# adobe-research/DiffusionHandles

Hardware: AMD Instinct MI355X
Metric: guided-denoise steps/sec at 512x512 (SD2-depth) (higher is better)
Workload: dtype f16; 1 GPU; single 512x512 edit per GPU, SD2-depth (865.9M params, seeded random weights), guided phase: 3 x (fwd + energy + bwd-to-latent) + CFG fwd (B=2) + DDIM step; resolution=512, edits_per_gpu=1, correspondences=24906, parallelism=independent edits, one process per GPU, no collectives

## Files before the change

diffusionhandles_amd/_lib.py:

```python
import ctypes
import os

import torch

_HERE = os.path.dirname(os.path.abspath(__file__))
LIB_PATH = os.environ.get("DIFFHANDLES_LIB") or os.path.join(_HERE, "libdiffhandles_hip.so")
_LIB = None

c_p = ctypes.c_void_p
c_i = ctypes.c_int
c_f = ctypes.c_float
c_d = ctypes.c_double
c_sz = ctypes.c_size_t


class UNetConfig(ctypes.Structure):
    _fields_ = [("in_channels", c_i), ("out_channels", c_i), ("n_levels", c_i),
                ("block_out_channels", c_i * 4), ("layers_per_block", c_i), ("heads", c_i * 4),
                ("cross_attention_dim", c_i), ("norm_groups", c_i), ("sample_size", c_i),
                ("text_len", c_i), ("max_batch", c_i), ("dtype", c_i), ("max_diff_batch", c_i)]


class VAEConfig(ctypes.Structure):
    _fields_ = [("latent_channels", c_i), ("out_channels", c_i), ("block_out_channels", c_i * 4),
# ... 97 lines not shown
    "dh_adam_step_scaled_batch": (c_i, [c_p, c_p, c_p, c_p, c_p, c_p, c_f, c_f, c_f, c_f, c_i, c_i, c_i, c_p]),
    "dh_latent_update_guarded": (c_i, [c_p, c_p, c_p, c_i, c_i, c_f, c_i, c_i, c_p, c_i, c_i, c_p, c_p, c_i, c_i, c_p]),
    "dh_ddim_cfg_step_flagged": (c_i, [c_p, c_p, c_p, c_p, c_f, c_f, c_f, c_i, c_i, c_p, c_i, c_i, c_p]),
}

c_l = ctypes.c_long
DEBUG_SIGNATURES = {
    "dh_dbg_gemm": (c_i, [c_i, c_p, c_l, c_p, c_i, c_i, c_i, c_i, c_i, c_i, c_i, c_i, c_i, c_i, c_i, c_p, c_p, c_i, c_i,
                          c_p, c_l, c_p, c_l, c_i, c_p, c_sz, c_p]),
    "dh_dbg_gemm_groupnorm": (c_i, [c_i, c_p, c_l, c_p, c_i, c_i, c_i, c_i, c_i, c_i, c_i, c_p, c_p, c_p, c_sz, c_i, c_i, c_p, c_p, c_f, c_i,
                                    c_p, c_p, c_p, ctypes.POINTER(c_i), c_p]),
    "dh_dbg_gemm_groupnorm_bwd": (c_i, [c_i, c_p, c_l, c_p, c_i, c_i, c_i, c_i, c_i, c_i, c_i, c_p, c_p, c_sz, c_i, c_i, c_p, c_p, c_p, c_p, c_i,
                                        c_p, c_p, ctypes.POINTER(c_i), c_p]),
    "dh_dbg_gemm_groupnorm_res": (c_i, [c_i, c_p, c_l, c_p, c_i, c_i, c_i, c_i, c_i, c_i, c_i, c_p, c_p, c_l, c_p, c_p, c_sz, c_i, c_i, c_p, c_p,
                                    c_f, c_i, c_p, c_p, c_p, ctypes.POINTER(c_i), c_p]),
    "dh_dbg_gemm_groupnorm_bwd_res": (c_i, [c_i, c_p, c_l, c_p, c_i, c_i, c_i, c_i, c_i, c_i, c_i, c_p, c_l, c_p, c_p, c_sz, c_i, c_i, c_p, c_p, c_p,
                                        c_p, c_i, c_p, c_p, ctypes.POINTER(c_i), c_p]),
    "dh_dbg_concat_groupnorm": (c_i, [c_i, c_p, c_i, c_p, c_i, c_p, c_i, c_i, c_i, c_p, c_p, c_f, c_i, c_p, c_p, c_p, c_p]),
    "dh_dbg_gemm_last_tile": (c_i, [ctypes.POINTER(c_i)]),
    "dh_dbg_unet_concat_ops": (c_i, [ctypes.POINTER(UNetConfig), ctypes.POINTER(c_i), c_i, ctypes.POINTER(c_i)]),
    "dh_dbg_gemm_lnfold": (c_i, [c_i, c_p, c_l, c_p, c_i, c_i, c_i, c_p, c_p, c_p, c_f, c_p, c_l, c_p]),
    "dh_dbg_gemm_glu": (c_i, [c_i, c_i, c_p, c_l, c_p, c_i, c_i, c_i, c_p, c_p, c_p, c_p, c_p, c_p]),
    "dh_dbg_gemm_glub_split": (c_i, [c_i, c_p, c_l, c_p, c_i, c_i, c_i, c_i, c_p, c_l, c_i, c_p, c_p, ctypes.POINTER(c_i), c_p]),
    "dh_dbg_unet_ff_fold": (c_i, [c_p, c_i, ctypes.POINTER(c_i), ctypes.POINTER(c_i), c_p, c_p, c_p]),
    "dh_dbg_gemm_family": (c_i, [c_i]),
    "dh_dbg_gemm_stage": (c_i, [c_i]),
    "dh_dbg_gemm_xattn": (c_i, [c_i, c_p, c_l, c_p, c_i, c_i, c_i, c_p, c_p, c_p, c_p, c_f, c_p, c_p, c_p, c_l, c_p, c_p, c_i, c_i, c_i,
                                ctypes.POINTER(c_i), c_p]),
    "dh_dbg_gemm_xattn_dq": (c_i, [c_i, c_p, c_l, c_p, c_i, c_i, c_i, c_p, c_p, c_p, c_p, c_l, c_p, c_p, c_p, c_i, c_i, ctypes.POINTER(c_i), c_p]),
    "dh_dbg_gemm_xattn_carried": (c_i, [ctypes.POINTER(c_i), ctypes.POINTER(ctypes.c_longlong)]),
    "dh_dbg_gemm_pp_variant": (c_i, [c_i, c_p]),
    "dh_dbg_gemm_pp_ablate": (c_i, [c_i]),
    "dh_dbg_gemm_pp_persist": (c_i, [c_i]),
    "dh_dbg_gemm_pp_glu": (c_i, [c_i]),
    "dh_dbg_gemm_pp_plan": (c_i, [c_i, c_i, c_i, c_i, c_i, c_i, c_sz, ctypes.POINTER(c_i), ctypes.POINTER(c_i), ctypes.POINTER(c_i)]),
    "dh_dbg_touch_tiled": (c_i, [c_sz, c_p]),
    "dh_dbg_groupnorm": (c_i, [c_i, c_p, c_p, c_p, c_p, c_p, c_p, c_p, c_p, c_i, c_i, c_i, c_i, c_f, c_i, c_i, c_p]),
    "dh_dbg_layernorm": (c_i, [c_i, c_p, c_p, c_p, c_p, c_p, c_p, c_p, c_p, c_i, c_i, c_f, c_p]),
    "dh_dbg_geglu": (c_i, [c_i, c_p, c_p, c_p, c_p, c_i, c_i, c_p]),
    "dh_dbg_attention": (c_i, [c_i, c_p, c_l, c_p, c_p, c_l, c_p, c_l, c_p, c_p, c_p, c_p, c_p, c_p, c_i, c_i, c_i, c_i, c_p]),
    "dh_dbg_attention_bwd_pair": (c_i, [c_i, c_p, c_l, c_p, c_p, c_l, c_p, c_l, c_p, c_p, c_p, c_p, c_p, c_p, c_i, c_i, c_i, c_i, c_p, c_p]),
    "dh_dbg_pool2x2": (c_i, [c_i, c_p, c_p, c_i, c_i, c_i, c_i, c_i, c_p]),
    "dh_dbg_ellipse_offsets": (c_i, [c_i, ctypes.POINTER(ctypes.c_int32), c_i, ctypes.POINTER(c_i)]),
    "dh_dbg_lane_ops": (c_i, [c_p, c_p, c_p, c_p]),
    "dh_dbg_cg_limits": (c_i, [ctypes.POINTER(c_i)]),
    "dh_dbg_cg_max_iter": (c_i, [c_i]),
}


def lib():
    global _LIB
    if _LIB is None:
        if not os.path.exists(LIB_PATH):
            raise RuntimeError(
                f"native HIP library not found at {LIB_PATH}; build it with "
                "`python -c 'import __graft_entry__ as g; g.build()'` (there is no CPU fallback)")
        handle = ctypes.CDLL(LIB_PATH)
        missing = []
        for name, (res, args) in list(SIGNATURES.items()) + list(DEBUG_SIGNATURES.items()):
            try:
# ... 38 lines not shown
```

diffusionhandles_amd/csrc/debug_api.cpp:

```cpp
#include <stdlib.h>

#include "unet_kernels.h"
using namespace dh;

static void* g_dbg_tiled = nullptr;

__global__ void k_dbg_touch(const uint4* p, size_t n16, unsigned* sink) {
  unsigned acc = 0;
  for (size_t i = (size_t)blockIdx.x * blockDim.x + threadIdx.x; i < n16; i += (size_t)gridDim.x * blockDim.x) { const uint4 v = p[i]; acc ^= v.x ^ v.y ^ v.z ^ v.w; }
  if (acc == 0x9e3779b9u && sink) sink[0] = acc;
}
extern "C" int dh_dbg_touch_tiled(size_t bytes, void* stream) {
  DH_REQUIRE(g_dbg_tiled != nullptr, "no tiled weights yet (call dh_dbg_gemm first)");
  hipLaunchKernelGGL(k_dbg_touch, dim3(512), dim3(256), 0, (hipStream_t)stream, (const uint4*)g_dbg_tiled, bytes / 16, (unsigned*)nullptr);
  DH_LAUNCH_CHECK();
  return DH_OK;
}

extern "C" int dh_dbg_gemm(int dtype, const void* A, long lda, const void* W, int M, int N, int K, int mode, int Hin,
                           int Win, int Cin, int Hout, int Wout, int stride, int up, const float* bias,
                           const float* rowvec, int rowvec_ld, int rows_per_batch, const void* R, long ldr, void* C,
                           long ldc, int act_silu, float* partial, size_t partial_elems, void* stream) {
  DH_REQUIRE(A && W && C && K % 64 == 0 && N % 64 == 0, "bad arguments (N, K must be multiples of 64)");
  void*& tiled = g_dbg_tiled;
// ... 197 lines not shown
  if (need > tiled_cap) {
    if (tiled) (void)hipFree(tiled);
    DH_CHECK_HIP(hipMalloc(&tiled, need));
    tiled_cap = need;
  }
  DH_CHECK_HIP(hipMemsetAsync(tiled, 0, need, (hipStream_t)stream));
  launch_tile_weights(dtype, W, tiled, N, K, (hipStream_t)stream);
  GemmArgs g;
  g.A = A; g.lda = lda; g.W = tiled; g.M = M; g.N = N; g.K = K; g.mode = A_DENSE;
  g.glub_x = x; g.glub_dx = dx; g.glub_f = F;
  g.C = C; g.ldc = ldc;
  if (accumulate) { g.R = C; g.ldr = ldc; }
  launch_gemm(dtype, g, (hipStream_t)stream);
  if (tile) dh_dbg_gemm_last_tile(tile);
  DH_LAUNCH_CHECK();
  return DH_OK;
}
extern "C" int dh_dbg_groupnorm(int dtype, const void* x, const float* gamma, const float* beta, void* y, float* stats,
                                const void* dy, void* dx, float* scratch, int B, int HW, int C, int G, float eps,
                                int silu, int accumulate, void* stream) {
  launch_groupnorm_fwd(dtype, x, gamma, beta, y, stats, scratch, B, HW, C, G, eps, silu, (hipStream_t)stream);
  if (dy && dx)
    launch_groupnorm_bwd(dtype, x, dy, gamma, beta, stats, dx, scratch, B, HW, C, G, silu, accumulate, (hipStream_t)stream);
  DH_LAUNCH_CHECK();
  return DH_OK;
}
extern "C" int dh_dbg_layernorm(int dtype, const void* x, const float* gamma, const float* beta, void* y, float* stats,
                                const void* dy, const void* add, void* dx, int rows, int C, float eps, void* stream) {
  launch_layernorm_fwd(dtype, x, gamma, beta, y, stats, rows, C, eps, (hipStream_t)stream);
  if (dy && dx) launch_layernorm_bwd(dtype, x, dy, gamma, stats, add, dx, rows, C, (hipStream_t)stream);
  DH_LAUNCH_CHECK();
  return DH_OK;
}
extern "C" int dh_dbg_geglu(int dtype, const void* x, void* y, const void* dy, void* dx, int rows, int F, void* stream) {
  launch_geglu_fwd(dtype, x, y, rows, F, (hipStream_t)stream);
  if (dy && dx) launch_geglu_bwd(dtype, x, dy, dx, rows, F, (hipStream_t)stream);
  DH_LAUNCH_CHECK();
  return DH_OK;
}
extern "C" int dh_dbg_attention(int dtype, const void* q, long ldq, const void* k, const void* v, long ldk, void* o,
                                long ldo, float* lse, const void* d_o, float* delta, void* dq, void* dk, void* dv,
                                int B, int H, int Nq, int Nk, void* stream) {
  hipStream_t st = (hipStream_t)stream;
  launch_attention_fwd(dtype, q, ldq, k, v, ldk, o, ldo, lse, B, H, Nq, Nk, st);
  if (d_o) {
    if (dq) launch_attention_bwd_dq(dtype, q, ldq, k, v, ldk, o, ldo, d_o, ldo, lse, delta, dq, ldq, B, H, Nq, Nk, st);
// ... 44 lines not shown
```

diffusionhandles_amd/csrc/gemm.hip:

```cpp
#include <stdlib.h>

#include <vector>

#include <hip/hip_ext.h>

#include "attn_tile.h"
#include "gemm_k.h"

namespace dh {

struct GemmProf {
  bool on = false;
  std::vector<hipEvent_t> ev;
  size_t used = 0;
  double flops = 0;
  double bytes = 0;
  hipEvent_t e0 = nullptr, e1 = nullptr;
};
static GemmProf g_prof;
static int g_buf_stage = 1;
static int g_pp_force = 0;
struct GemmTileReport {
  int bm, bn, kg, stages, mw, splits, pp, gn_epi, reduce_gn;
};
static thread_local GemmTileReport g_last_tile;
static thread_local int g_last_xattn = 0;
static thread_local long long g_xattn_total = 0;
#ifdef DH_TUNING
static unsigned long long* g_gemm_ts = nullptr;
#endif
bool gemm_profiling_on() { return g_prof.on; }

constexpr int BK = 64;
#ifdef DH_EXP_SETPRIO
#define DH_PRIO(x) __builtin_amdgcn_s_setprio(x)
#else
#define DH_PRIO(x) do { } while (0)
#endif


template <class T>
__device__ __forceinline__ uint2 epilogue_pack(const GemmK& p, int m, int n, float v0, float v1, float v2, float v3,
                                               bool have_r, uint2 rpre, bool have_b, float4 bpre) {
  float v[4] = {v0, v1, v2, v3};
  if (p.bias) {
    float4 b = bpre;
    if (!have_b) b = *reinterpret_cast<const float4*>(p.bias + n);
    v[0] += b.x; v[1] += b.y; v[2] += b.z; v[3] += b.w;
  }
  if (p.rowvec) {
    const float4 b = *reinterpret_cast<const float4*>(p.rowvec + (size_t)div_small(m, p.inv_rows_per_batch) * p.rowvec_ld + n);
    v[0] += b.x; v[1] += b.y; v[2] += b.z; v[3] += b.w;
  }
  if (p.act_silu) {
// ... 1585 lines not shown
```

diffusionhandles_amd/csrc/unet_engine.cpp:

```cpp
#include <stdlib.h>

#include <algorithm>
#include <map>
#include <numeric>
#include <vector>

#include "unet_kernels.h"

namespace dh {

enum OpType { OP_CONV_IN, OP_CONV_OUT, OP_GEMM, OP_GN, OP_LN, OP_ATTN, OP_GEGLU, OP_CONCAT, OP_TIMESTEP, OP_T2F };
enum ParamKind { PK_F32, PK_MAT };

struct Ten {
  size_t off = 0, goff = 0;
  size_t off_fo = 0;
  int rows = 0, C = 0;
  int ld = 0;
  int view = -1, col = 0;
  bool req_grad = true;
  bool persistent = false;
};

struct Wt {
// ... 66 lines not shown
  hipStream_t temb_stream = nullptr;
  uint64_t text_key = 0, kv_key = 0;
  int kv_rows = 0;
  hipStream_t kv_stream = nullptr;
  long temb_f32_off = -1;
  int temb_total = 0, kv_total = 0;
  float *in_sample = nullptr, *in_text = nullptr, *io_eps = nullptr, *out_dsample = nullptr, *out_dtext = nullptr, *t_dev = nullptr;
  std::map<uint64_t, hipGraphExec_t> graphs;
  std::map<uint64_t, double> graph_flops;
  bool use_graphs = true;
  long ones_off = -1, zeros_off = -1;
  bool fold_dirty = true;
  bool owns_weights = true;
  int n_shared = 0;
  int saved_batch = 0;
  const float* saved_sample = nullptr;
  std::vector<char> gready;
  double flops_fwd = 0, flops_bwd = 0;
  int64_t launches = 0;

  bool fo_mode = false;
  unsigned short* aptr(int t, int B_unused = 0) { return act + (fo_mode && !tens[t].persistent ? tens[t].off_fo : tens[t].off); }
  std::vector<int> galias;
  unsigned short* gptr(int t) {
    while (galias[t] != t) t = galias[t];
    return grad + tens[t].goff;
  }
};

namespace {

struct Builder {
  dh_unet& u;
  int maxB, maxBd;
  explicit Builder(dh_unet& uu) : u(uu), maxB(uu.cfg.max_batch), maxBd(uu.cfg.max_diff_batch) {}

  int tensor(int rows, int C, bool req_grad = true) {
    Ten t;
    t.rows = rows; t.C = C; t.ld = C; t.req_grad = req_grad;
    u.tens.push_back(t);
    return (int)u.tens.size() - 1;
  }
  void set_view(int t, int root, int col) {
    Ten& tt = u.tens[t];
    tt.view = root; tt.col = col; tt.ld = u.tens[root].C;
  }
// ... 928 lines not shown

namespace {
struct Bwd {
  dh_unet* u;
  int B, dt;
  hipStream_t st;
  bool need_text;
  void add_into(int t, const unsigned short* src, long lds_, int cols, int col_off = 0) {
    const Ten& tt = u->tens[t];
    launch_copy_cols(dt, src, lds_, u->gptr(t) + col_off, tt.C, B * tt.rows, cols, u->gready[t] ? 1 : 0, st);
  }
};
}

static void backward_ops(dh_unet* u, int B, unsigned act_mask, bool has_eps, bool want_sample, bool want_text,
                         hipStream_t st) {
  const int dt = u->dtype;
  const dh_unet_config& c = u->cfg;
  const float* d_eps = has_eps ? u->io_eps : nullptr;
  float* d_sample = want_sample ? u->out_dsample : nullptr;
  float* d_text = want_text ? u->out_dtext : nullptr;
  u->flops_bwd = 0;
  std::fill(u->gready.begin(), u->gready.end(), 0);
  for (int i = 0; i < 3; ++i)
    if (act_mask & (1u << i)) u->gready[u->act_ids[i]] = 1;
  Bwd bw{u, B, dt, st, d_text != nullptr};
  bool text_grad_written = false;
  int gnb_have = 0, gnb_for = -1;
  int lnb_have = 0, lnb_for = -1;
  int cat_done = -1;
  int glub_done = -1;
  int xb_have = 0, xb_for = -1;
  for (int oi = (int)u->ops.size() - 1; oi >= 0; --oi) {
    const Op& o = u->ops[oi];
    if (!want_sample && oi < u->first_cross_op && o.out != u->t_kv) continue;
    switch (o.type) {
      case OP_CONV_OUT: {
        if (!d_eps) break;
        const Wt& w = u->wts[o.wt];
        launch_conv_small_bwd(dt, d_eps, 1, u->pf + w.bwd_off, u->gptr(o.in0), 0, 0, B, o.Hin, o.Hin, w.N, o.Cin, st);
        u->gready[o.in0] = 1;
        u->flops_bwd += 2.0 * B * o.Hin * o.Hin * w.N * w.K;
        break;
      }
      case OP_CONV_IN: {
        if (!d_sample || !u->gready[o.out]) break;
        const Wt& w = u->wts[o.wt];
        launch_conv_small_bwd(dt, u->gptr(o.out), 0, u->pf + w.bwd_off, d_sample, 1, 0, B, o.Hin, o.Hin, w.N, o.Cin, st);
        u->flops_bwd += 2.0 * B * o.Hin * o.Hin * w.N * w.K;
        break;
      }
      case OP_GEMM: {
        if (!u->tens[o.out].req_grad || !u->gready[o.out]) break;
        const Ten& to = u->tens[o.out];
        const Ten& ti = u->tens[o.in0];
        const Wt& w = u->wts[o.wt];
        if (o.res >= 0 && u->tens[o.res].req_grad) {
          if (u->gready[o.res]) bw.add_into(o.res, u->gptr(o.out), to.C, to.C);
          else u->galias[o.res] = o.out;
          u->gready[o.res] = 1;
        }
        if (o.glub_op >= 0 && o.in1 >= 0) {
          const Op& ge = u->ops[o.glub_op];
          const int t2 = o.in1;
          GemmArgs g;
          g.A = u->gptr(o.out); g.lda = to.C;
          g.W = u->w16 + w.bwd_off;
          g.mode = A_DENSE; g.M = B * to.rows; g.N = w.K; g.K = w.N;
          g.partial = u->partial; g.partial_elems = u->partial_elems;
          g.glub_x = u->aptr(ge.in0); g.glub_dx = u->gptr(ge.in0); g.glub_f = u->tens[ge.out].C;
          g.C = u->gptr(t2); g.ldc = u->tens[t2].C;
          if (u->gready[t2]) { g.R = g.C; g.ldr = g.ldc; }
          u->flops_bwd += launch_gemm(dt, g, st);
          u->gready[ge.in0] = 1; u->gready[ge.out] = 1; u->gready[t2] = 1;
          glub_done = o.glub_op;
          break;
        }
        if (!ti.req_grad || !w.has_bwd) break;
        if (o.in0 == u->t_text && !bw.need_text) break;
        GemmArgs g;
        g.A = u->gptr(o.out); g.lda = to.C;
        g.W = u->w16 + w.bwd_off;
// ... 54 lines not shown
          if (u->gready[o.in0]) { g.R = g.C; g.ldr = ti.C; }
          gnb_have = 0;
          int gi = -1;
          if (oi > 0 && u->ops[oi - 1].type == OP_GN && u->ops[oi - 1].out == o.in0) gi = oi - 1;
          else if (oi > 1 && u->ops[oi - 1].type == OP_GEMM && u->ops[oi - 1].mode == A_DENSE && u->ops[oi - 1].out == o.res &&
                   u->ops[oi - 1].in0 != o.in0 && u->ops[oi - 2].type == OP_GN && u->ops[oi - 2].out == o.in0)
            gi = oi - 2;
          if (gi >= 0) {
            const Op& gn = u->ops[gi];
            const Ten& tx = u->tens[gn.in0];
            g.gnb_x = u->aptr(gn.in0); g.gnb_ldx = tx.ld;
            g.gnb_gamma = u->pf + gn.gamma_off; g.gnb_beta = u->pf + gn.beta_off; g.gnb_stats = u->f32a + gn.stats_off;
            g.gnb_silu = gn.silu;
            g.gn_part = u->small; g.gn_HW = tx.rows; g.gn_G = gn.groups; g.gn_done = &gnb_have;
            gnb_for = gi;
          }
          u->flops_bwd += launch_gemm(dt, g, st);
          u->gready[o.in0] = 1;
        }
        if (o.in0 == u->t_text) text_grad_written = true;
        break;
      }
      case OP_GN: {
        if (!u->gready[o.out]) break;
        const Ten& t = u->tens[o.in0];
        GnBwdSplit split;
        if (oi > 0 && u->ops[oi - 1].type == OP_CONCAT && u->ops[oi - 1].out == o.in0) {
          const Op& cat = u->ops[oi - 1];
          const int ca = u->tens[cat.in0].C;
          if (!u->gready[cat.in0] && !u->gready[cat.in1] && ca % 8 == 0 && ca + u->tens[cat.in1].C == t.C) {
            split.out0 = u->gptr(cat.in0); split.out1 = u->gptr(cat.in1); split.split_c = ca;
            cat_done = oi - 1;
          }
        }
        launch_groupnorm_bwd(dt, u->aptr(o.in0), u->gptr(o.out), u->pf + o.gamma_off, u->pf + o.beta_off,
                             u->f32a + o.stats_off, u->gptr(o.in0), u->small, B, t.rows, t.C, o.groups, o.silu,
                             u->gready[o.in0] ? 1 : 0, st, gnb_for == oi ? gnb_have : 0, split);
        gnb_have = 0;
        u->gready[o.in0] = 1;
        if (split.out0) { u->gready[u->ops[oi - 1].in0] = 1; u->gready[u->ops[oi - 1].in1] = 1; }
        break;
      }
      case OP_LN: {
        if (!u->gready[o.out]) break;
        if (lnb_have && lnb_for == oi) {
          lnb_have = 0;
          u->gready[o.in0] = 1;
          break;
        }
        const Ten& t = u->tens[o.in0];
        launch_layernorm_bwd(dt, u->aptr(o.in0), u->gptr(o.out), u->pf + o.gamma_off, u->f32a + o.stats_off,
                             u->gready[o.in0] ? u->gptr(o.in0) : nullptr, u->gptr(o.in0), B * t.rows, t.C, st, t.ld);
        u->gready[o.in0] = 1;
        break;
      }
      case OP_GEGLU: {
        if (!u->gready[o.out]) break;
        if (glub_done == oi) { glub_done = -1; break; }
        const Ten& t = u->tens[o.out];
        launch_geglu_bwd(dt, u->aptr(o.in0), u->gptr(o.out), u->gptr(o.in0), B * t.rows, t.C, st);
// ... 132 lines not shown
  DH_REQUIRE(cfg && n_out && (out || cap == 0), "null pointer");
  dh_unet u;
  u.cfg = *cfg;
  const int rc = build(u);
  if (rc != DH_OK) return rc;
  int n = 0;
  for (size_t i = 0; i < u.ops.size(); ++i) {
    const Op& o = u.ops[i];
    if (o.type != OP_CONCAT) continue;
    const Ten &a = u.tens[o.in0], &b = u.tens[o.in1], &t = u.tens[o.out];
    const int G = o.gn_next >= 0 ? u.ops[o.gn_next].groups : 0;
    const bool fused = o.gn_next >= 0 && i + 1 < u.ops.size() && a.C % 8 == 0 && b.C % 8 == 0 && t.C % G == 0 &&
                       (GN_GB * (t.C / G)) % 8 == 0 && GN_GB * (t.C / G) <= 2048;
    if (n < cap) {
      int* e = out + 5 * n;
      e[0] = a.C; e[1] = b.C; e[2] = t.rows; e[3] = G; e[4] = fused ? 1 : 0;
    }
    ++n;
  }
  *n_out = n;
  return DH_OK;
}

extern "C" int dh_dbg_unet_ff_fold(dh_unet* u, int i, int* n_folds, int* C, void* w, float* bias, void* stream) {
  DH_REQUIRE(u && n_folds && C, "null pointer");
  hipStream_t st = (hipStream_t)stream;
  *n_folds = (int)u->ffolds.size();
  *C = 0;
  if (i < 0 || i >= (int)u->ffolds.size()) return DH_OK;
  if (u->fold_dirty) fold_layernorms(u, st);
  const FfFold& f = u->ffolds[i];
  const Wt& wf = u->wts[f.wt];
  *C = wf.N;
  if (w)
    hipLaunchKernelGGL((k_untile<unsigned short>), dim3(cdiv(wf.N * wf.K, 256)), dim3(256), 0, st,
                       (const unsigned short*)(u->w16 + wf.fwd_off), wf.N, wf.K, (unsigned short*)w);
  if (bias) DH_CHECK_HIP(hipMemcpyAsync(bias, u->pf + f.bias, (size_t)wf.N * 4, hipMemcpyDeviceToDevice, st));
  DH_LAUNCH_CHECK();
  return DH_OK;
}
```

diffusionhandles_amd/csrc/unet_kernels.h:

```cpp
#pragma once
#include "common.h"

namespace dh {

__device__ inline float silu_grad(float z) {
  const float s = 1.f / (1.f + __expf(-z));
  return s * (1.f + z * (1.f - s));
}

struct GeluParts { float Phi, pdf; };
__device__ __forceinline__ GeluParts gelu_parts(float g) {
  const float x = fabsf(g) * 0.70710678118654752f;
  const float t = __builtin_amdgcn_rcpf(fmaf(0.3275911f, x, 1.f));
  const float e = __expf(-x * x);
  const float poly = t * (0.254829592f + t * (-0.284496736f + t * (1.421413741f + t * (-1.453152027f + t * 1.061405429f))));
  const float q = 0.5f * poly * e;
  return {g < 0.f ? q : 1.f - q, e * 0.3989422804014327f};
}
__device__ __forceinline__ float gelu_f(float g) { return g * gelu_parts(g).Phi; }
__device__ __forceinline__ float gelu_grad(float g) { const GeluParts p = gelu_parts(g); return fmaf(g, p.pdf, p.Phi); }
__host__ __device__ inline int glu_col(int o, int gate) { return 32 * (o >> 4) + 16 * gate + (o & 15); }
__host__ __device__ inline int glu_src_row(int n, int F) { return ((n >> 4) & 1) * F + 16 * (n >> 5) + (n & 15); }

enum { A_DENSE = 0, A_CONV3 = 1, A_CONVT2 = 2 };
// ... 9 lines not shown
  int pad = 1;
  const float* bias = nullptr;
  const float* rowvec = nullptr; int rowvec_ld = 0; int rows_per_batch = 1;
  const void* R = nullptr; long ldr = 0;
  void* C = nullptr; long ldc = 0;
  int act_silu = 0;
  float* partial = nullptr; size_t partial_elems = 0;
  float* gn_part = nullptr; int gn_HW = 0, gn_G = 0; int* gn_done = nullptr;
  const void* gnb_x = nullptr; long gnb_ldx = 0; const float *gnb_gamma = nullptr, *gnb_beta = nullptr, *gnb_stats = nullptr;
  int gnb_silu = 0;
  const float* ln_s = nullptr; const float* ln_t = nullptr; float* ln_stats = nullptr; float ln_eps = 1e-5f;
  const void* lnb_x = nullptr; long lnb_ldx = 0; const float *lnb_gamma = nullptr, *lnb_stats = nullptr; const void* lnb_add = nullptr;
  void* lnb_dx = nullptr; int* lnb_done = nullptr;
  void* glu_y = nullptr; long glu_ldy = 0;
  const void* glub_x = nullptr; void* glub_dx = nullptr; int glub_f = 0;
  const void *xa_k = nullptr, *xa_v = nullptr; long xa_ldk = 0; void* xa_o = nullptr; long xa_ldo = 0; float* xa_lse = nullptr;
  int xa_H = 0, xa_Nq = 0, xa_Nk = 0, xa_save = 1; int* xa_done = nullptr;
  const void* xa_q = nullptr; long xa_ldq = 0; void* xa_dq = nullptr; long xa_lddq = 0;
};
void launch_splitk_reduce_ln_bwd(int dtype, const float* partial, int splits, const void* x, const float* gamma,
                                 const float* stats, const void* add, void* dx, int rows, int C, hipStream_t st, long ldx = 0);
double launch_gemm(int dtype, const GemmArgs& a, hipStream_t st);
bool gemm_profiling_on();
void launch_tile_weights(int dtype, const void* src, void* dst, int N, int K, hipStream_t st, int conv_cin = 0);
__host__ __device__ inline size_t wt_index(int n, int k, int K) {
  const int r = n & 63, c = (k & 63) >> 3;
  return ((size_t)(n >> 6) * (K >> 6) + (k >> 6)) * 4096 + (size_t)r * 64 + (size_t)((c ^ ((r >> 1) & 7)) << 3) + (k & 7);
}

__host__ __device__ inline int conv_k_index(int tap, int c) { return (c >> 6) * 576 + tap * 64 + (c & 63); }

void launch_load_weight(int dtype, const float* src, int N, int C, int taps, void* fwd, long fwd_K, long row_off, void* bwd,
                        long bwd_K, long col_off, int Nb, float scale, hipStream_t st);

void launch_conv_small_fwd(int dtype, const void* x, int x_is_f32, const float* w, const float* bias, void* y,
                           int y_is_f32, int B, int H, int W, int Cin, int Cout, hipStream_t st);
void launch_conv_small_bwd(int dtype, const void* dy, int dy_is_f32, const float* w, void* dx, int dx_is_f32,
                           int accumulate, int B, int H, int W, int Cin, int Cout, hipStream_t st);

void launch_groupnorm_fwd(int dtype, const void* x, const float* gamma, const float* beta, void* y, float* stats,
                          float* scratch, int B, int HW, int C, int G, float eps, int silu, hipStream_t st,
                          int have_partials = 0);
int gn_slices(int HW, int B);
constexpr int GN_GB = 4;
void launch_concat_gn(int dtype, const void* a, int Ca, const void* b, int Cb, void* out, float* gn_part, int B, int HW,
                      int G, hipStream_t st);
struct GnBwdSplit { void* out0 = nullptr; void* out1 = nullptr; int split_c = 0; };
void launch_groupnorm_bwd(int dtype, const void* x, const void* dy, const float* gamma, const float* beta,
                          const float* stats, void* dx, float* scratch, int B, int HW, int C, int G, int silu,
                          int accumulate, hipStream_t st, int have_partials = 0, GnBwdSplit split = GnBwdSplit());
void launch_gelu(int dtype, const void* x, void* y, size_t n, hipStream_t st);
void launch_layernorm_fwd(int dtype, const void* x, const float* gamma, const float* beta, void* y, float* stats,
                          int rows, int C, float eps, hipStream_t st, long ldx = 0);
void launch_layernorm_bwd(int dtype, const void* x, const void* dy, const float* gamma, const float* stats,
                          const void* add, void* dx, int rows, int C, hipStream_t st, long ldx = 0);
void launch_geglu_fwd(int dtype, const void* x, void* y, int rows, int F, hipStream_t st);
void launch_geglu_bwd(int dtype, const void* x, const void* dy, void* dx, int rows, int F, hipStream_t st);
void launch_copy_cols(int dtype, const void* src, long lds, void* dst, long ldd, int rows, int cols, int accumulate,
                      hipStream_t st);
void launch_split_cols(int dtype, const void* src, long lds, void* dstA, long ldA, int colsA, int accA, void* dstB, long ldB,
                       int colsB, int accB, int rows, hipStream_t st);
void launch_lane_ops_probe(const float* in, float* out, unsigned* ex, hipStream_t st);
void launch_pool2x2_sum(int dtype, const void* src, void* dst, int B, int h, int w, int C, int accumulate,
                        hipStream_t st);
void launch_f32_to_t(int dtype, const float* src, void* dst, size_t n, hipStream_t st);
void launch_t_to_f32(int dtype, const void* src, float* dst, size_t n, int accumulate, hipStream_t st);
void launch_timestep_embedding(int dtype, const float* t_dev, int dim, int B, void* out, hipStream_t st);
void launch_set_scalar(float* p, float v, hipStream_t st);

void launch_attention_fwd(int dtype, const void* q, long ldq, const void* k, const void* v, long ldk, void* o,
                          long ldo, float* lse, int B, int H, int Nq, int Nk, hipStream_t st, int causal = 0);
void launch_attention_delta(int dtype, const void* o, long ldo, const void* d_o, long lddo, float* delta, int B,
                            int H, int Nq, hipStream_t st);
// ... 10 lines not shown
```

diffusionhandles_amd/csrc/unet_kernels.hip:

```cpp
#include "unet_kernels.h"

namespace dh {

#ifdef DH_TUNING
static int ablate_mask() { static const int m = getenv("DH_ABLATE_SKIP") ? atoi(getenv("DH_ABLATE_SKIP")) : 0; return m; }
__global__ void k_noop() {}
static int ablate_empty() { static const int m = getenv("DH_ABLATE_EMPTY") ? atoi(getenv("DH_ABLATE_EMPTY")) : 0; return m; }
#define DH_ABLATE(bit) do { if (ablate_mask() & (bit)) { if (ablate_empty()) hipLaunchKernelGGL(k_noop, dim3(1), dim3(64), 0, st); return; } } while (0)
#else
#define DH_ABLATE(bit) do { } while (0)
#endif

constexpr int CF_PIX = 4;
template <class T>
__global__ void k_conv_few_in(const float* x, const float* w, const float* bias, T* y, int B, int H, int W, int Ci,
                              int Co) {
  __shared__ float patch[CF_PIX][9 * 8];
  const int K = 9 * Ci, total = B * H * W;
  const int p0 = blockIdx.x * CF_PIX;
  for (int i = threadIdx.x; i < CF_PIX * K; i += blockDim.x) {
    const int lp = i / K, k = i - lp * K, p = p0 + lp;
    float v = 0.f;
    if (p < total) {
      const int b = p / (H * W), r = p - b * H * W, oy = r / W, ox = r - oy * W;
// ... 244 lines not shown
  m2 = oct_sum(m2);
  m2 = m2 > 0.f ? m2 : 0.f;
  if (act && sub == 0) {
    const float rstd = rsqrtf(m2 / n + eps);
    sm_stats[g] = make_float2(mean, rstd);
    if (stats_out) { stats_out[2 * (b * G + g)] = mean; stats_out[2 * (b * G + g) + 1] = rstd; }
  }
  __syncthreads();
}

template <class T, bool WIDE>
__global__ void __launch_bounds__(256) k_gn_apply(const T* x, const float* gamma, const float* beta, const float* part,
                                                  float* stats, T* y, int HW, int C, int G, int S, float eps, int silu,
                                                  int iters) {
  __shared__ float2 sm_stats[64];
  const int b = blockIdx.y;
  const int cchunks = C / 8, cpg = C / G;
  const float inv_cpg = 1.f / (float)cpg;
  const unsigned total = (unsigned)HW * cchunks;
  unsigned idx = blockIdx.x * iters * blockDim.x + threadIdx.x;
  bool live = idx < total;
  unsigned pix = live ? idx / cchunks : 0;
  size_t row = (size_t)b * HW + pix;
  int c0 = (int)(idx - pix * cchunks) * 8;
  uint4 raw = *reinterpret_cast<const uint4*>(x + row * C + c0);
  float gmv[8], btv[8];
  *reinterpret_cast<float4*>(gmv) = *reinterpret_cast<const float4*>(gamma + c0);
  *reinterpret_cast<float4*>(gmv + 4) = *reinterpret_cast<const float4*>(gamma + c0 + 4);
  *reinterpret_cast<float4*>(btv) = *reinterpret_cast<const float4*>(beta + c0);
  *reinterpret_cast<float4*>(btv + 4) = *reinterpret_cast<const float4*>(beta + c0 + 4);
  gn_combine(part, b, G, S, eps, sm_stats, blockIdx.x == 0 ? stats : nullptr);
  for (int it = 0; it < iters; ++it) {
    if (!live) return;
    uint4 nraw = raw;
    float ngm[8], nbt[8];
    const unsigned nidx = idx + blockDim.x;
    const bool nlive = it + 1 < iters && nidx < total;
    size_t nrow = row;
    int nc0 = c0;
    if (nlive) {
      const unsigned npix = nidx / cchunks;
      nrow = (size_t)b * HW + npix;
      nc0 = (int)(nidx - npix * cchunks) * 8;
      nraw = *reinterpret_cast<const uint4*>(x + nrow * C + nc0);
      *reinterpret_cast<float4*>(ngm) = *reinterpret_cast<const float4*>(gamma + nc0);
      *reinterpret_cast<float4*>(ngm + 4) = *reinterpret_cast<const float4*>(gamma + nc0 + 4);
      *reinterpret_cast<float4*>(nbt) = *reinterpret_cast<const float4*>(beta + nc0);
// ... 23 lines not shown
  size_t it = blocks_total / 1024;
  return it < 1 ? 1 : (it > 8 ? 8 : (int)it);
}

void launch_groupnorm_fwd(int dtype, const void* x, const float* gamma, const float* beta, void* y, float* stats,
                          float* scratch, int B, int HW, int C, int G, float eps, int silu, hipStream_t st,
                          int have_partials) {
  DH_ABLATE(2);
  const int S = have_partials > 1 ? have_partials : gn_slices(HW, B);
  const size_t blocks0 = ((size_t)HW * (C / 8) + 255) / 256;
  const int iters = gn_apply_iters(blocks0 * B);
  dim3 g1(S, cdiv(G, GN_GB), B), g2((unsigned)((blocks0 + iters - 1) / iters), B);
  if (dtype == DH_DTYPE_F16) {
    if (!have_partials) hipLaunchKernelGGL((k_gn_partial<f16, false>), g1, dim3(256), 0, st, (const f16*)x, (const f16*)nullptr, gamma, beta, (const float*)nullptr, scratch, HW, C, G, S, silu);
    if (C / G >= 8) hipLaunchKernelGGL((k_gn_apply<f16, true>), g2, dim3(256), 0, st, (const f16*)x, gamma, beta, scratch, stats, (f16*)y, HW, C, G, S, eps, silu, iters);
    else hipLaunchKernelGGL((k_gn_apply<f16, false>), g2, dim3(256), 0, st, (const f16*)x, gamma, beta, scratch, stats, (f16*)y, HW, C, G, S, eps, silu, iters);
  } else {
    if (!have_partials) hipLaunchKernelGGL((k_gn_partial<bf16, false>), g1, dim3(256), 0, st, (const bf16*)x, (const bf16*)nullptr, gamma, beta, (const float*)nullptr, scratch, HW, C, G, S, silu);
    if (C / G >= 8) hipLaunchKernelGGL((k_gn_apply<bf16, true>), g2, dim3(256), 0, st, (const bf16*)x, gamma, beta, scratch, stats, (bf16*)y, HW, C, G, S, eps, silu, iters);
    else hipLaunchKernelGGL((k_gn_apply<bf16, false>), g2, dim3(256), 0, st, (const bf16*)x, gamma, beta, scratch, stats, (bf16*)y, HW, C, G, S, eps, silu, iters);
  }
}

template <class T, bool WIDE>
__global__ void __launch_bounds__(256) k_gn_bwd_apply(const T* x, const T* dy, const float* gamma, const float* beta,
                                                      const float* stats, const float* part, T* dx, int HW, int C, int G,
                                                      int S, int silu, int accumulate, int iters, T* split0, T* split1,
                                                      int split_c) {
  __shared__ float4 sm_st[64];
  const int b = blockIdx.y, cpg = C / G;
  const float inv_cpg = 1.f / (float)cpg;
  const int cchunks = C / 8;
  const unsigned total = (unsigned)HW * cchunks;
  unsigned idx = blockIdx.x * iters * blockDim.x + threadIdx.x;
  bool live = idx < total;
  unsigned pix = live ? idx / cchunks : 0;
  size_t row = (size_t)b * HW + pix;
  int c0 = (int)(idx - pix * cchunks) * 8;
  uint4 rx = *reinterpret_cast<const uint4*>(x + row * C + c0);
  uint4 rd = *reinterpret_cast<const uint4*>(dy + row * C + c0);
  uint4 ro = make_uint4(0, 0, 0, 0);
  if (accumulate) ro = *reinterpret_cast<const uint4*>(dx + row * C + c0);
  float gmv[8], btv[8];
  *reinterpret_cast<float4*>(gmv) = *reinterpret_cast<const float4*>(gamma + c0);
  *reinterpret_cast<float4*>(gmv + 4) = *reinterpret_cast<const float4*>(gamma + c0 + 4);
  *reinterpret_cast<float4*>(btv) = *reinterpret_cast<const float4*>(beta + c0);
  *reinterpret_cast<float4*>(btv + 4) = *reinterpret_cast<const float4*>(beta + c0 + 4);
  {
    const int g = threadIdx.x >> 3, sub = threadIdx.x & 7;
    const bool act = g < G;
    const float2* p = reinterpret_cast<const float2*>(part) + (size_t)(b * G + (act ? g : 0)) * S;
    float2 v[GN_COMBINE_K];
#pragma unroll
    for (int k = 0; k < GN_COMBINE_K; ++k) {
      const int s = sub + 8 * k;
      v[k] = act && s < S ? p[s] : make_float2(0.f, 0.f);
    }
    float2 st = act ? *reinterpret_cast<const float2*>(stats + 2 * (b * G + g)) : make_float2(0.f, 0.f);
    float a = 0.f, c = 0.f;
#pragma unroll
    for (int k = 0; k < GN_COMBINE_K; ++k) { a += v[k].x; c += v[k].y; }
    a = oct_sum(a); c = oct_sum(c);
    const float inv = 1.f / ((float)HW * (float)cpg);
    if (act && sub == 0) sm_st[g] = make_float4(st.x, st.y, a * inv, c * inv);
  }
  __syncthreads();
  typedef T T8 __attribute__((ext_vector_type(8)));
  for (int it = 0; it < iters; ++it) {
    if (!live) return;
    const unsigned nidx = idx + blockDim.x;
    const bool nlive = it + 1 < iters && nidx < total;
    size_t nrow = row;
    int nc0 = c0;
    uint4 nrx = rx, nrd = rd, nro = ro;
    float ngm[8], nbt[8];
    if (nlive) {
      const unsigned npix = nidx / cchunks;
      nrow = (size_t)b * HW + npix;
      nc0 = (int)(nidx - npix * cchunks) * 8;
      nrx = *reinterpret_cast<const uint4*>(x + nrow * C + nc0);
      nrd = *reinterpret_cast<const uint4*>(dy + nrow * C + nc0);
      if (accumulate) nro = *reinterpret_cast<const uint4*>(dx + nrow * C + nc0);
      *reinterpret_cast<float4*>(ngm) = *reinterpret_cast<const float4*>(gamma + nc0);
      *reinterpret_cast<float4*>(ngm + 4) = *reinterpret_cast<const float4*>(gamma + nc0 + 4);
      *reinterpret_cast<float4*>(nbt) = *reinterpret_cast<const float4*>(beta + nc0);
      *reinterpret_cast<float4*>(nbt + 4) = *reinterpret_cast<const float4*>(beta + nc0 + 4);
    }
    const T8 xv = __builtin_bit_cast(T8, rx), dv = __builtin_bit_cast(T8, rd), ov = __builtin_bit_cast(T8, ro);
    T8 o;
    const int g0 = (int)(((float)c0 + 0.5f) * inv_cpg), bnd = (g0 + 1) * cpg - c0;
    const float4 st0 = sm_st[g0], st1 = sm_st[g0 + 1 < G ? g0 + 1 : g0];
#pragma unroll
    for (int i = 0; i < 8; ++i) {
      const float4 st = WIDE ? (i < bnd ? st0 : st1) : sm_st[(c0 + i) / cpg];
      const float xh = (to_f32<T>(xv[i]) - st.x) * st.y;
      float d = to_f32<T>(dv[i]);
      if (silu) d *= silu_grad(xh * gmv[i] + btv[i]);
      d *= gmv[i];
      float r = st.y * (d - st.z - xh * st.w);
      if (accumulate) r += to_f32<T>(ov[i]);
      o[i] = from_f32<T>(r);
    }
    T* dst = !split0 ? dx + row * C + c0
                     : (c0 < split_c ? split0 + row * split_c + c0 : split1 + row * (C - split_c) + (c0 - split_c));
    *reinterpret_cast<uint4*>(dst) = __builtin_bit_cast(uint4, o);
    if (!nlive) return;
    idx = nidx; row = nrow; c0 = nc0; rx = nrx; rd = nrd; ro = nro;
#pragma unroll
    for (int i = 0; i < 8; ++i) { gmv[i] = ngm[i]; btv[i] = nbt[i]; }
  }
}

void launch_groupnorm_bwd(int dtype, const void* x, const void* dy, const float* gamma, const float* beta,
                          const float* stats, void* dx, float* scratch, int B, int HW, int C, int G, int silu,
                          int accumulate, hipStream_t st, int have_partials, GnBwdSplit split) {
  DH_ABLATE(2);
  const int S = have_partials > 1 ? have_partials : gn_slices(HW, B);
  const size_t blocks0 = ((size_t)HW * (C / 8) + 255) / 256;
  const int iters = gn_apply_iters(blocks0 * B);
  dim3 g1(S, cdiv(G, GN_GB), B), g2((unsigned)((blocks0 + iters - 1) / iters), B);
  if (dtype == DH_DTYPE_F16) {
    if (!have_partials) hipLaunchKernelGGL((k_gn_partial<f16, true>), g1, dim3(256), 0, st, (const f16*)x, (const f16*)dy, gamma, beta, stats, scratch, HW, C, G, S, silu);
    if (C / G >= 8) hipLaunchKernelGGL((k_gn_bwd_apply<f16, true>), g2, dim3(256), 0, st, (const f16*)x, (const f16*)dy, gamma, beta, stats, scratch, (f16*)dx, HW, C, G, S, silu, accumulate, iters, (f16*)split.out0, (f16*)split.out1, split.split_c);
    else hipLaunchKernelGGL((k_gn_bwd_apply<f16, false>), g2, dim3(256), 0, st, (const f16*)x, (const f16*)dy, gamma, beta, stats, scratch, (f16*)dx, HW, C, G, S, silu, accumulate, iters, (f16*)split.out0, (f16*)split.out1, split.split_c);
  } else {
    if (!have_partials) hipLaunchKernelGGL((k_gn_partial<bf16, true>), g1, dim3(256), 0, st, (const bf16*)x, (const bf16*)dy, gamma, beta, stats, scratch, HW, C, G, S, silu);
    if (C / G >= 8) hipLaunchKernelGGL((k_gn_bwd_apply<bf16, true>), g2, dim3(256), 0, st, (const bf16*)x, (const bf16*)dy, gamma, beta, stats, scratch, (bf16*)dx, HW, C, G, S, silu, accumulate, iters, (bf16*)split.out0, (bf16*)split.out1, split.split_c);
    else hipLaunchKernelGGL((k_gn_bwd_apply<bf16, false>), g2, dim3(256), 0, st, (const bf16*)x, (const bf16*)dy, gamma, beta, stats, scratch, (bf16*)dx, HW, C, G, S, silu, accumulate, iters, (bf16*)split.out0, (bf16*)split.out1, split.split_c);
  }
}

template <class T>
__global__ void __launch_bounds__(256) k_concat_gn(const T* a, int Ca, const T* bsrc, int Cb, T* out, float* part, int HW, int G,
                                                   int S) {
  __shared__ float sm_red[4][2 * GN_GB];
  const int C = Ca + Cb;
  const int s = blockIdx.x, g0 = blockIdx.y * GN_GB, b = blockIdx.z, cpg = div_small(C, rcp_fast(G));
  const int W = GN_GB * cpg, nch = W >> 3;
  const float inv_nch = rcp_fast(nch), inv_S = rcp_fast(S);
  const int RP = div_small((int)blockDim.x, inv_nch);
  const int r0 = div_small(HW * s, inv_S), r1 = div_small(HW * (s + 1), inv_S);
  const int rr = div_small((int)threadIdx.x, inv_nch), ch = threadIdx.x - rr * nch;
  auto load8 = [&](size_t m, int n) {
    return n < Ca ? *reinterpret_cast<const uint4*>(a + m * Ca + n) : *reinterpret_cast<const uint4*>(bsrc + m * Cb + (n - Ca));
  };
  float ga[GN_GB], gq[GN_GB], pg[GN_GB];
#pragma unroll
  for (int gl = 0; gl < GN_GB; ++gl) {
    ga[gl] = 0.f; gq[gl] = 0.f; pg[gl] = 0.f;
    if (g0 + gl < G) {
      const int n = (g0 + gl) * cpg;
// ... 553 lines not shown
```

Before: 38.53 steps/s.

## Defer residual-gradient add into the following GroupNorm backward apply kernel

During the UNet backward pass, a residual-branch gradient that would have been added into a tensor with a separate add kernel is now deferred when the next op touching that tensor is a GroupNorm on it. The GroupNorm backward apply kernel gains a templated extra addend input and folds the residual gradient in while writing dx. This saves one read-modify-write pass over the activation gradient per residual block. The cost is an extra kernel variant, some bookkeeping for pending addends, and a fallback copy when the GroupNorm gradient turns out not to be needed.

Result: no change. 38.60 steps/s, median of 6 (+0.2%).

```diff
diff --git a/diffusionhandles_amd/_lib.py b/diffusionhandles_amd/_lib.py
--- a/diffusionhandles_amd/_lib.py
+++ b/diffusionhandles_amd/_lib.py
@@ -143,6 +143,7 @@
     "dh_dbg_gemm_lnfold": (c_i, [c_i, c_p, c_l, c_p, c_i, c_i, c_i, c_p, c_p, c_p, c_f, c_p, c_l, c_p]),
     "dh_dbg_gemm_glu": (c_i, [c_i, c_i, c_p, c_l, c_p, c_i, c_i, c_i, c_p, c_p, c_p, c_p, c_p, c_p]),
     "dh_dbg_gemm_glub_split": (c_i, [c_i, c_p, c_l, c_p, c_i, c_i, c_i, c_i, c_p, c_l, c_i, c_p, c_p, ctypes.POINTER(c_i), c_p]),
+    "dh_dbg_unet_gn_addends": (c_i, [c_p, ctypes.POINTER(c_i), ctypes.POINTER(c_i)]),
     "dh_dbg_unet_ff_fold": (c_i, [c_p, c_i, ctypes.POINTER(c_i), ctypes.POINTER(c_i), c_p, c_p, c_p]),
     "dh_dbg_gemm_family": (c_i, [c_i]),
     "dh_dbg_gemm_stage": (c_i, [c_i]),
@@ -157,6 +158,8 @@
     "dh_dbg_gemm_pp_plan": (c_i, [c_i, c_i, c_i, c_i, c_i, c_i, c_sz, ctypes.POINTER(c_i), ctypes.POINTER(c_i), ctypes.POINTER(c_i)]),
     "dh_dbg_touch_tiled": (c_i, [c_sz, c_p]),
     "dh_dbg_groupnorm": (c_i, [c_i, c_p, c_p, c_p, c_p, c_p, c_p, c_p, c_p, c_i, c_i, c_i, c_i, c_f, c_i, c_i, c_p]),
+    "dh_dbg_groupnorm_bwd_addend": (c_i, [c_i, c_p, c_p, c_p, c_p, c_p, c_p, c_p, c_i, c_i, c_i, c_i, c_i, c_i, c_p, c_l, c_p, c_p, c_i,
+                                          c_i, c_p]),
     "dh_dbg_layernorm": (c_i, [c_i, c_p, c_p, c_p, c_p, c_p, c_p, c_p, c_p, c_i, c_i, c_f, c_p]),
     "dh_dbg_geglu": (c_i, [c_i, c_p, c_p, c_p, c_p, c_i, c_i, c_p]),
     "dh_dbg_attention": (c_i, [c_i, c_p, c_l, c_p, c_p, c_l, c_p, c_l, c_p, c_p, c_p, c_p, c_p, c_p, c_i, c_i, c_i, c_i, c_p]),
diff --git a/diffusionhandles_amd/csrc/debug_api.cpp b/diffusionhandles_amd/csrc/debug_api.cpp
--- a/diffusionhandles_amd/csrc/debug_api.cpp
+++ b/diffusionhandles_amd/csrc/debug_api.cpp
@@ -243,6 +243,22 @@
   launch_groupnorm_fwd(dtype, x, gamma, beta, y, stats, scratch, B, HW, C, G, eps, silu, (hipStream_t)stream);
   if (dy && dx)
     launch_groupnorm_bwd(dtype, x, dy, gamma, beta, stats, dx, scratch, B, HW, C, G, silu, accumulate, (hipStream_t)stream);
+  DH_LAUNCH_CHECK();
+  return DH_OK;
+}
+extern "C" int dh_dbg_groupnorm_bwd_addend(int dtype, const void* x, const void* dy, const float* gamma, const float* beta,
+                                           const float* stats, void* dx, float* scratch, int B, int HW, int C, int G, int silu,
+                                           int accumulate, const void* add, long ld_add, void* split0, void* split1, int split_c,
+                                           int fused, void* stream) {
+  DH_REQUIRE(x && dy && gamma && beta && stats && dx && scratch && add && C % 8 == 0 && ld_add % 8 == 0 && ld_add >= C, "bad arguments");
+  GnBwdSplit split;
+  split.out0 = split0; split.out1 = split1; split.split_c = split_c;
+  if (fused) {
+    launch_groupnorm_bwd(dtype, x, dy, gamma, beta, stats, dx, scratch, B, HW, C, G, silu, accumulate, (hipStream_t)stream, 0, split, add, ld_add);
+  } else {
+    launch_copy_cols(dtype, add, ld_add, dx, C, B * HW, C, accumulate, (hipStream_t)stream);
+    launch_groupnorm_bwd(dtype, x, dy, gamma, beta, stats, dx, scratch, B, HW, C, G, silu, 1, (hipStream_t)stream, 0, split);
+  }
   DH_LAUNCH_CHECK();
   return DH_OK;
 }
diff --git a/diffusionhandles_amd/csrc/gemm.hip b/diffusionhandles_amd/csrc/gemm.hip
--- a/diffusionhandles_amd/csrc/gemm.hip
+++ b/diffusionhandles_amd/csrc/gemm.hip
@@ -30,6 +30,7 @@
 static unsigned long long* g_gemm_ts = nullptr;
 #endif
 bool gemm_profiling_on() { return g_prof.on; }
+int gemm_debug_bits() { return g_buf_stage; }
 
 constexpr int BK = 64;
 #ifdef DH_EXP_SETPRIO
diff --git a/diffusionhandles_amd/csrc/unet_engine.cpp b/diffusionhandles_amd/csrc/unet_engine.cpp
--- a/diffusionhandles_amd/csrc/unet_engine.cpp
+++ b/diffusionhandles_amd/csrc/unet_engine.cpp
@@ -112,6 +112,8 @@
   bool fo_mode = false;
   unsigned short* aptr(int t, int B_unused = 0) { return act + (fo_mode && !tens[t].persistent ? tens[t].off_fo : tens[t].off); }
   std::vector<int> galias;
+  std::vector<int> gpend;
+  int gn_addends = 0, res_copies = 0;
   unsigned short* gptr(int t) {
     while (galias[t] != t) t = galias[t];
     return grad + tens[t].goff;
@@ -1086,6 +1088,9 @@
   float* d_text = want_text ? u->out_dtext : nullptr;
   u->flops_bwd = 0;
   std::fill(u->gready.begin(), u->gready.end(), 0);
+  u->gpend.assign(u->tens.size(), -1);
+  u->gn_addends = 0; u->res_copies = 0;
+  const bool gn_addend = (gemm_debug_bits() & 64) == 0;
   for (int i = 0; i < 3; ++i)
     if (act_mask & (1u << i)) u->gready[u->act_ids[i]] = 1;
   Bwd bw{u, B, dt, st, d_text != nullptr};
@@ -1120,8 +1125,18 @@
         const Ten& ti = u->tens[o.in0];
         const Wt& w = u->wts[o.wt];
         if (o.res >= 0 && u->tens[o.res].req_grad) {
-          if (u->gready[o.res]) bw.add_into(o.res, u->gptr(o.out), to.C, to.C);
-          else u->galias[o.res] = o.out;
+          if (u->gready[o.res]) {
+            int next = oi - 1;
+            while (next >= 0) {
+              const Op& q = u->ops[next];
+              if (q.in0 == o.res || q.in1 == o.res || q.res == o.res || q.out == o.res) break;
+              --next;
+            }
+            const bool by_gn = gn_addend && next >= 0 && u->ops[next].type == OP_GN && u->ops[next].in0 == o.res &&
+                               u->tens[o.res].C == to.C && u->gpend[o.res] < 0 && (want_sample || next >= u->first_cross_op);
+            if (by_gn) u->gpend[o.res] = o.out;
+            else { bw.add_into(o.res, u->gptr(o.out), to.C, to.C); ++u->res_copies; }
+          } else u->galias[o.res] = o.out;
           u->gready[o.res] = 1;
         }
         if (o.glub_op >= 0 && o.in1 >= 0) {
@@ -1222,7 +1237,13 @@
         break;
       }
       case OP_GN: {
-        if (!u->gready[o.out]) break;
+        const int pend = u->gpend[o.in0];
+        u->gpend[o.in0] = -1;
+        if (!u->gready[o.out]) {
+          if (pend >= 0) { bw.add_into(o.in0, u->gptr(pend), u->tens[pend].C, u->tens[pend].C); ++u->res_copies; }
+          break;
+        }
+        if (pend >= 0) ++u->gn_addends;
         const Ten& t = u->tens[o.in0];
         GnBwdSplit split;
         if (oi > 0 && u->ops[oi - 1].type == OP_CONCAT && u->ops[oi - 1].out == o.in0) {
@@ -1235,7 +1256,8 @@
         }
         launch_groupnorm_bwd(dt, u->aptr(o.in0), u->gptr(o.out), u->pf + o.gamma_off, u->pf + o.beta_off,
                              u->f32a + o.stats_off, u->gptr(o.in0), u->small, B, t.rows, t.C, o.groups, o.silu,
-                             u->gready[o.in0] ? 1 : 0, st, gnb_for == oi ? gnb_have : 0, split);
+                             u->gready[o.in0] ? 1 : 0, st, gnb_for == oi ? gnb_have : 0, split,
+                             pend >= 0 ? u->gptr(pend) : nullptr, pend >= 0 ? u->tens[pend].C : 0);
         gnb_have = 0;
         u->gready[o.in0] = 1;
         if (split.out0) { u->gready[u->ops[oi - 1].in0] = 1; u->gready[u->ops[oi - 1].in1] = 1; }
@@ -1414,6 +1436,13 @@
   return DH_OK;
 }
 
+extern "C" int dh_dbg_unet_gn_addends(const dh_unet* u, int* addends, int* copies) {
+  DH_REQUIRE(u && addends && copies, "null pointer");
+  *addends = u->gn_addends;
+  *copies = u->res_copies;
+  return DH_OK;
+}
+
 extern "C" int dh_dbg_unet_ff_fold(dh_unet* u, int i, int* n_folds, int* C, void* w, float* bias, void* stream) {
   DH_REQUIRE(u && n_folds && C, "null pointer");
   hipStream_t st = (hipStream_t)stream;
diff --git a/diffusionhandles_amd/csrc/unet_kernels.h b/diffusionhandles_amd/csrc/unet_kernels.h
--- a/diffusionhandles_amd/csrc/unet_kernels.h
+++ b/diffusionhandles_amd/csrc/unet_kernels.h
@@ -55,6 +55,7 @@
                                  const float* stats, const void* add, void* dx, int rows, int C, hipStream_t st, long ldx = 0);
 double launch_gemm(int dtype, const GemmArgs& a, hipStream_t st);
 bool gemm_profiling_on();
+int gemm_debug_bits();
 void launch_tile_weights(int dtype, const void* src, void* dst, int N, int K, hipStream_t st, int conv_cin = 0);
 __host__ __device__ inline size_t wt_index(int n, int k, int K) {
   const int r = n & 63, c = (k & 63) >> 3;
@@ -81,7 +82,8 @@
 struct GnBwdSplit { void* out0 = nullptr; void* out1 = nullptr; int split_c = 0; };
 void launch_groupnorm_bwd(int dtype, const void* x, const void* dy, const float* gamma, const float* beta,
                           const float* stats, void* dx, float* scratch, int B, int HW, int C, int G, int silu,
-                          int accumulate, hipStream_t st, int have_partials = 0, GnBwdSplit split = GnBwdSplit());
+                          int accumulate, hipStream_t st, int have_partials = 0, GnBwdSplit split = GnBwdSplit(),
+                          const void* add2 = nullptr, long ld2 = 0);
 void launch_gelu(int dtype, const void* x, void* y, size_t n, hipStream_t st);
 void launch_layernorm_fwd(int dtype, const void* x, const float* gamma, const float* beta, void* y, float* stats,
                           int rows, int C, float eps, hipStream_t st, long ldx = 0);
diff --git a/diffusionhandles_amd/csrc/unet_kernels.hip b/diffusionhandles_amd/csrc/unet_kernels.hip
--- a/diffusionhandles_amd/csrc/unet_kernels.hip
+++ b/diffusionhandles_amd/csrc/unet_kernels.hip
@@ -290,7 +290,7 @@
   bool live = idx < total;
   unsigned pix = live ? idx / cchunks : 0;
   size_t row = (size_t)b * HW + pix;
-  int c0 = (int)(idx - pix * cchunks) * 8;
+  int c0 = live ? (int)(idx - pix * cchunks) * 8 : 0;
   uint4 raw = *reinterpret_cast<const uint4*>(x + row * C + c0);
   float gmv[8], btv[8];
   *reinterpret_cast<float4*>(gmv) = *reinterpret_cast<const float4*>(gamma + c0);
@@ -360,11 +360,11 @@
   }
 }
 
-template <class T, bool WIDE>
+template <class T, bool WIDE, bool ADD2>
 __global__ void __launch_bounds__(256) k_gn_bwd_apply(const T* x, const T* dy, const float* gamma, const float* beta,
                                                       const float* stats, const float* part, T* dx, int HW, int C, int G,
                                                       int S, int silu, int accumulate, int iters, T* split0, T* split1,
-                                                      int split_c) {
+                                                      int split_c, const T* add2, long ld2) {
   __shared__ float4 sm_st[64];
   const int b = blockIdx.y, cpg = C / G;
   const float inv_cpg = 1.f / (float)cpg;
@@ -374,11 +374,13 @@
   bool live = idx < total;
   unsigned pix = live ? idx / cchunks : 0;
   size_t row = (size_t)b * HW + pix;
-  int c0 = (int)(idx - pix * cchunks) * 8;
+  int c0 = live ? (int)(idx - pix * cchunks) * 8 : 0;
   uint4 rx = *reinterpret_cast<const uint4*>(x + row * C + c0);
   uint4 rd = *reinterpret_cast<const uint4*>(dy + row * C + c0);
   uint4 ro = make_uint4(0, 0, 0, 0);
   if (accumulate) ro = *reinterpret_cast<const uint4*>(dx + row * C + c0);
+  uint4 ra = make_uint4(0, 0, 0, 0);
+  if (ADD2) ra = *reinterpret_cast<const uint4*>(add2 + row * ld2 + c0);
   float gmv[8], btv[8];
   *reinterpret_cast<float4*>(gmv) = *reinterpret_cast<const float4*>(gamma + c0);
   *reinterpret_cast<float4*>(gmv + 4) = *reinterpret_cast<const float4*>(gamma + c0 + 4);
@@ -410,7 +412,7 @@
     const bool nlive = it + 1 < iters && nidx < total;
     size_t nrow = row;
     int nc0 = c0;
-    uint4 nrx = rx, nrd = rd, nro = ro;
+    uint4 nrx = rx, nrd = rd, nro = ro, nra = ra;
     float ngm[8], nbt[8];
     if (nlive) {
       const unsigned npix = nidx / cchunks;
@@ -419,12 +421,14 @@
       nrx = *reinterpret_cast<const uint4*>(x + nrow * C + nc0);
       nrd = *reinterpret_cast<const uint4*>(dy + nrow * C + nc0);
       if (accumulate) nro = *reinterpret_cast<const uint4*>(dx + nrow * C + nc0);
+      if (ADD2) nra = *reinterpret_cast<const uint4*>(add2 + nrow * ld2 + nc0);
       *reinterpret_cast<float4*>(ngm) = *reinterpret_cast<const float4*>(gamma + nc0);
       *reinterpret_cast<float4*>(ngm + 4) = *reinterpret_cast<const float4*>(gamma + nc0 + 4);
       *reinterpret_cast<float4*>(nbt) = *reinterpret_cast<const float4*>(beta + nc0);
       *reinterpret_cast<float4*>(nbt + 4) = *reinterpret_cast<const float4*>(beta + nc0 + 4);
     }
     const T8 xv = __builtin_bit_cast(T8, rx), dv = __builtin_bit_cast(T8, rd), ov = __builtin_bit_cast(T8, ro);
+    const T8 av = __builtin_bit_cast(T8, ra);
     T8 o;
     const int g0 = (int)(((float)c0 + 0.5f) * inv_cpg), bnd = (g0 + 1) * cpg - c0;
     const float4 st0 = sm_st[g0], st1 = sm_st[g0 + 1 < G ? g0 + 1 : g0];
@@ -435,23 +439,41 @@
       float d = to_f32<T>(dv[i]);
       if (silu) d *= silu_grad(xh * gmv[i] + btv[i]);
       d *= gmv[i];
-      float r = st.y * (d - st.z - xh * st.w);
-      if (accumulate) r += to_f32<T>(ov[i]);
+      const float t = d - st.z - xh * st.w;
+      float r = st.y * t;
+      if (ADD2) {
+        const float base = accumulate ? to_f32<T>(from_f32<T>(to_f32<T>(av[i]) + to_f32<T>(ov[i]))) : to_f32<T>(av[i]);
+        r = fmaf(st.y, t, base);
+        asm volatile("" : "+v"(r));
+      } else if (accumulate) r += to_f32<T>(ov[i]);
       o[i] = from_f32<T>(r);
     }
     T* dst = !split0 ? dx + row * C + c0
                      : (c0 < split_c ? split0 + row * split_c + c0 : split1 + row * (C - split_c) + (c0 - split_c));
     *reinterpret_cast<uint4*>(dst) = __builtin_bit_cast(uint4, o);
     if (!nlive) return;
-    idx = nidx; row = nrow; c0 = nc0; rx = nrx; rd = nrd; ro = nro;
+    idx = nidx; row = nrow; c0 = nc0; rx = nrx; rd = nrd; ro = nro; ra = nra;
 #pragma unroll
     for (int i = 0; i < 8; ++i) { gmv[i] = ngm[i]; btv[i] = nbt[i]; }
   }
+}
+
+template <class T>
+static void gn_bwd_apply_launch(dim3 grid, hipStream_t st, const void* x, const void* dy, const float* gamma, const float* beta,
+                                const float* stats, float* scratch, void* dx, int HW, int C, int G, int S, int silu,
+                                int accumulate, int iters, const GnBwdSplit& split, const void* add2, long ld2) {
+#define DH_GNB(WIDE, ADD2)                                                                                                    \
+  hipLaunchKernelGGL((k_gn_bwd_apply<T, WIDE, ADD2>), grid, dim3(256), 0, st, (const T*)x, (const T*)dy, gamma, beta, stats, \
+                     scratch, (T*)dx, HW, C, G, S, silu, accumulate, iters, (T*)split.out0, (T*)split.out1, split.split_c,   \
+                     (const T*)add2, ld2)
+  if (C / G >= 8) { if (add2) DH_GNB(true, true); else DH_GNB(true, false); }
+  else { if (add2) DH_GNB(false, true); else DH_GNB(false, false); }
+#undef DH_GNB
 }
 
 void launch_groupnorm_bwd(int dtype, const void* x, const void* dy, const float* gamma, const float* beta,
                           const float* stats, void* dx, float* scratch, int B, int HW, int C, int G, int silu,
-                          int accumulate, hipStream_t st, int have_partials, GnBwdSplit split) {
+                          int accumulate, hipStream_t st, int have_partials, GnBwdSplit split, const void* add2, long ld2) {
   DH_ABLATE(2);
   const int S = have_partials > 1 ? have_partials : gn_slices(HW, B);
   const size_t blocks0 = ((size_t)HW * (C / 8) + 255) / 256;
@@ -459,12 +481,10 @@
   dim3 g1(S, cdiv(G, GN_GB), B), g2((unsigned)((blocks0 + iters - 1) / iters), B);
   if (dtype == DH_DTYPE_F16) {
     if (!have_partials) hipLaunchKernelGGL((k_gn_partial<f16, true>), g1, dim3(256), 0, st, (const f16*)x, (const f16*)dy, gamma, beta, stats, scratch, HW, C, G, S, silu);
-    if (C / G >= 8) hipLaunchKernelGGL((k_gn_bwd_apply<f16, true>), g2, dim3(256), 0, st, (const f16*)x, (const f16*)dy, gamma, beta, stats, scratch, (f16*)dx, HW, C, G, S, silu, accumulate, iters, (f16*)split.out0, (f16*)split.out1, split.split_c);
-    else hipLaunchKernelGGL((k_gn_bwd_apply<f16, false>), g2, dim3(256), 0, st, (const f16*)x, (const f16*)dy, gamma, beta, stats, scratch, (f16*)dx, HW, C, G, S, silu, accumulate, iters, (f16*)split.out0, (f16*)split.out1, split.split_c);
+    gn_bwd_apply_launch<f16>(g2, st, x, dy, gamma, beta, stats, scratch, dx, HW, C, G, S, silu, accumulate, iters, split, add2, ld2);
   } else {
     if (!have_partials) hipLaunchKernelGGL((k_gn_partial<bf16, true>), g1, dim3(256), 0, st, (const bf16*)x, (const bf16*)dy, gamma, beta, stats, scratch, HW, C, G, S, silu);
-    if (C / G >= 8) hipLaunchKernelGGL((k_gn_bwd_apply<bf16, true>), g2, dim3(256), 0, st, (const bf16*)x, (const bf16*)dy, gamma, beta, stats, scratch, (bf16*)dx, HW, C, G, S, silu, accumulate, iters, (bf16*)split.out0, (bf16*)split.out1, split.split_c);
-    else hipLaunchKernelGGL((k_gn_bwd_apply<bf16, false>), g2, dim3(256), 0, st, (const bf16*)x, (const bf16*)dy, gamma, beta, stats, scratch, (bf16*)dx, HW, C, G, S, silu, accumulate, iters, (bf16*)split.out0, (bf16*)split.out1, split.split_c);
+    gn_bwd_apply_launch<bf16>(g2, st, x, dy, gamma, beta, stats, scratch, dx, HW, C, G, S, silu, accumulate, iters, split, add2, ld2);
   }
 }
 
```
